# usamireko/WFL-ASR

Hardware: AMD Instinct MI355X
Metric: audio_seconds_labeled_per_sec_per_node (higher is better)
Workload: dtype bf16; 1 GPU; BASELINE configs[1]: openai/whisper-base + 2 Conformer blocks, 16 x 30 s clips per GPU; clips_per_gpu=16, frames_per_clip=1500, tags=141, parallelism=clip-sharded dp1, launch=eager, batches_in_flight=2

## Files before the change

wfl-asr_amd/csrc/gemm_stream.hip:

```cpp
#include "common.h"
#include <cstdlib>
#include <cstring>
#include <type_traits>

#define SBK 32
#ifndef SNST
#define SNST 4
#endif

#ifndef SNCU
#define SNCU 256
#endif

typedef __attribute__((address_space(1))) const void* sgptr_t;
typedef __attribute__((address_space(3))) void* slptr_t;
typedef __attribute__((ext_vector_type(2))) __bf16 bf16x2;

static __device__ __forceinline__ void sglds(const bf16_t* g, char* l) {
  __builtin_amdgcn_global_load_lds((sgptr_t)g, (slptr_t)l, 16, 0, 0);
}
static __device__ __forceinline__ int sswz(int row) { return (-(row >> 2)) & 3; }
static __device__ __forceinline__ int xswz(int row) { return ((row >> 2) & 1) << 1; }
template <int N>
static __device__ __forceinline__ void wait_vm() { asm volatile("s_waitcnt vmcnt(%0)" ::"n"(N) : "memory"); }

#ifdef WFL_GEMM_STAMPS
#define SSTAMP(k) do { if (tid == 0 && p.stamps) { p.stamps[(long)blockIdx.x * 8 + (k)] = __builtin_amdgcn_s_memrealtime(); \
    if ((k) == 1) p.stamps[(long)blockIdx.x * 8 + 5] = __builtin_amdgcn_s_memtime(); \
    if ((k) == 2) p.stamps[(long)blockIdx.x * 8 + 6] = __builtin_amdgcn_s_memtime(); } } while (0)
#else
#define SSTAMP(k) do { } while (0)
#endif

template <int ACT, int MT, bool RES, int LNF, bool STATS, bool CONV, bool W8 = false, bool A8 = false, bool OUT8 = false, bool NOLO = false>
__global__ __launch_bounds__(512) void gemm_stream_kernel(GemmArgs p) {
  static_assert(!NOLO || CONV, "only the conv mode has an optional low half");
  static_assert(!CONV || (MT == 6 && !RES && LNF == 0 && !STATS), "conv mode: 192-row tiles, plain epilogue");
  static_assert(!W8 || (!CONV && MT == 6), "fp8 weights: plain 192-row mode");
  static_assert(!A8 || (!W8 && !CONV && MT == 6 && LNF == 0 && !STATS), "fp8 x fp8: the plain 192-row mode, no LayerNorm folding");
  static_assert(!OUT8 || (A8 && !RES), "fp8 output: the fp8 x fp8 kernel, no residual");
  constexpr int BMV = MT * 32;
#ifdef WFL_LAB_STB32
  constexpr int STB = 512 * SBK * 2;
  constexpr int WOFF = 256 * SBK * 2;
#else
  constexpr int STB = CONV ? 256 * SBK * 2 : BMV * SBK * 2 + 256 * SBK * (W8 ? 1 : 2);
  constexpr int WOFF = CONV ? 0 : BMV * SBK * 2;
#endif
  constexpr int AEXT = 224 * SBK * 2;
  constexpr int AOFF = SNST * STB;
  constexpr bool LOUT = RES || (CONV && !NOLO);
  constexpr int NSTORE = (LOUT ? 4 : 2) * MT + (STATS ? MT : 0);
  constexpr int SROW = 4;
  extern __shared__ __attribute__((aligned(16))) char smem[];
  float* stat_lds = (float*)(smem + SNST * STB + (CONV ? 2 * AEXT : 0));
  const int tid = threadIdx.x;
  const int lane = tid & 63;
  const int wid = __builtin_amdgcn_readfirstlane(tid >> 6);
  const int grp = wid >> 2, wq = wid & 3;
  const int g = lane >> 4, c = lane & 15;
  const int G = gridDim.x;

  SSTAMP(0);
  const int tiles_n = p.N / 256;
  const int tiles_m = (p.M + BMV - 1) / BMV;
  const int ntiles = tiles_m * tiles_n;
  const int nk = p.K / SBK;
  auto tile_of = [&](int v, int& m0, int& n0) __attribute__((always_inline)) {
    const int q = ntiles >> 3, r = ntiles & 7, x = v & 7, i = v >> 3;
    const int bid = (x < r ? x * (q + 1) : r * (q + 1) + (x - r) * q) + i;
    const int tm = bid / tiles_n;
    m0 = tm * BMV;
    n0 = (bid - tm * tiles_n) * 256;
  };
  const int wm = grp * (MT * 16), wn = wq * 64;

  const bool two_x = CONV ? wid < 6 : (MT == 8 || wid < 4);
  const int xg0 = CONV ? (wid < 6 ? wid * 2 : 12 + (wid - 6)) : ((MT == 8 || wid < 4) ? wid * 2 : 8 + (wid - 4));
  const int ntaps = CONV ? (p.tap_wrap > 0 ? p.tap_wrap : p.K / p.cin) : 1;
  const int nchunk = CONV ? p.cin / SBK : 1;
  const bf16_t* a_src[2];
  const bf16_t* w_src[2];
  const char* w8_src = nullptr;
  int pv = blockIdx.x, pkt = 0, issued = 0;
  int islot = 0;
  int ptap_k = 0;
  long pbase = 0;
  int ptap_i = 0, pseg = 0;
  auto next_tap = [&]() __attribute__((always_inline)) {
    ptap_k = 0;
    if (p.tap_wrap > 0 && ++ptap_i == p.tap_wrap) { ptap_i = 0; ++pseg; pbase = pseg == 1 ? p.seg_off : 0; }
    else pbase += p.tap_stride;
  };
  int pcc = 0, ptap = 0, pccg = 0;
  long pa_off = 0, pw_off = 0;
  auto set_src = [&](int v) __attribute__((always_inline)) {
    int m0, n0;
    tile_of(v, m0, n0);
    int lane = tid & 63;
    asm volatile("" : "+v"(lane));
#pragma unroll
    for (int i = 0; i < 2; ++i) {
      const int wrow = (wid * 2 + i) * 16 + (lane >> 2);
      const int xrow = (xg0 + i) * 16 + (lane >> 2);
      int am = m0 + xrow;
      const int am_max = CONV ? p.M - 1 + ntaps - 1 : p.M - 1;
      am = am < am_max ? am : am_max;
      a_src[i] = p.A + (long)am * p.lda + ((lane & 3) ^ (CONV ? xswz(xrow) : sswz(xrow))) * 8;
      w_src[i] = p.W + (long)(n0 + wrow) * p.K + ((lane & 3) ^ sswz(wrow)) * 8;
    }
    if (W8) {
      const int Gr = wid * 4 + (lane >> 4);
      const int ul = (lane & 15) ^ ((Gr & 1) | (((Gr >> 1) & 1) << 3));
      w8_src = (const char*)p.W + (long)(n0 + 8 * Gr + (ul >> 1)) * p.K + (ul & 1) * 16;
    }
  };
  set_src(pv);
  auto issue_stage = [&]() __attribute__((always_inline)) {
    if (CONV) {
      char* base = smem + islot * STB;
      islot = islot + 1 == SNST ? 0 : islot + 1;
      if (ptap == 0) {
        char* ab = smem + AOFF + (pccg & 1) * AEXT;
        sglds(a_src[0] + pa_off, ab + xg0 * 1024);
        if (two_x) sglds(a_src[1] + pa_off, ab + xg0 * 1024 + 1024);
      }
#pragma unroll
      for (int i = 0; i < 2; ++i) sglds(w_src[i] + ptap * p.cin + pw_off, base + wid * 2048 + i * 1024);
      ++issued;
      ++pkt;
      if (++ptap == ntaps) {
        ptap = 0; ++pcc; ++pccg;
        if (pcc == nchunk) { pcc = 0; ++pseg; }
        pa_off = (pseg == 1 ? p.seg_off : 0) + (long)pcc * SBK;
        pw_off = (long)pseg * ntaps * p.cin + (long)pcc * SBK;
      }
      return;
    }
    const long koff = pbase + ptap_k;
    char* base = smem + islot * STB;
    islot = islot + 1 == SNST ? 0 : islot + 1;
    sglds(a_src[0] + koff, base + xg0 * 1024);
    if (two_x) sglds(a_src[1] + koff, base + xg0 * 1024 + 1024);
    if (W8) {
      sglds((const bf16_t*)(w8_src + pkt * SBK), base + WOFF + wid * 1024);
    } else {
#pragma unroll
      for (int i = 0; i < 2; ++i) sglds(w_src[i] + pkt * SBK, base + WOFF + wid * 2048 + i * 1024);
    }
    ++issued;
    ++pkt;
    ptap_k += SBK;
    if (ptap_k == p.cin) next_tap();
  };
  int d_pkt = 0;
  char* d_base = nullptr;
  auto issue_stage_split = [&](auto ndc_c) __attribute__((always_inline)) {
    constexpr int NDC = decltype(ndc_c)::value;
    const long koff = pbase + ptap_k;
    char* base = smem + islot * STB;
    islot = islot + 1 == SNST ? 0 : islot + 1;
    sglds(a_src[0] + koff, base + xg0 * 1024);
    if (two_x) sglds(a_src[1] + koff, base + xg0 * 1024 + 1024);
    if (W8) {
      if (NDC == 0) sglds((const bf16_t*)(w8_src + pkt * SBK), base + WOFF + wid * 1024);
    } else {
#pragma unroll
      for (int i = 0; i < 2 - NDC; ++i) sglds(w_src[i] + pkt * SBK, base + WOFF + wid * 2048 + i * 1024);
    }
    d_pkt = pkt; d_base = base;
    ++issued;
    ++pkt;
    ptap_k += SBK;
    if (ptap_k == p.cin) next_tap();
  };
  auto issue_deferred = [&](int j, auto ndc_c) __attribute__((always_inline)) {
    constexpr int NDC = decltype(ndc_c)::value;
    if (W8) sglds((const bf16_t*)(w8_src + d_pkt * SBK), d_base + WOFF + wid * 1024);
    else sglds(w_src[2 - NDC + j] + d_pkt * SBK, d_base + WOFF + wid * 2048 + (2 - NDC + j) * 1024);
  };
  auto prefetch_one = [&]() __attribute__((always_inline)) {
    if (pv >= ntiles) return;
    issue_stage();
    if (pkt == nk) {
      pkt = 0; ptap_k = 0; pbase = 0; pcc = 0; ptap = 0; ptap_i = 0; pseg = 0; pa_off = 0; pw_off = 0;
      pv += G;
      if (pv < ntiles) set_src(pv);
    }
  };
  auto wait_stage = [&](int need, bool with_stores) __attribute__((always_inline)) {
    const int younger = issued - need - 1;
    if (younger < 0) return;
    constexpr int L2X = CONV ? 2 : (W8 ? 3 : 4), L1X = CONV ? 2 : (W8 ? 2 : 3);
    static_assert(SNST >= 3 && SNST <= 6, "ring depth");
#define WFL_WAITY(L)                                                                              \
    do {                                                                                          \
      if (SNST >= 6 && younger >= 4) { if (with_stores) wait_vm<4 * (L) + NSTORE>(); else wait_vm<4 * (L)>(); }       \
      else if (SNST >= 5 && younger >= 3) { if (with_stores) wait_vm<3 * (L) + NSTORE>(); else wait_vm<3 * (L)>(); }  \
      else if (younger >= 2) { if (with_stores) wait_vm<2 * (L) + NSTORE>(); else wait_vm<2 * (L)>(); }              \
      else if (younger == 1) { if (with_stores) wait_vm<(L) + NSTORE>(); else wait_vm<(L)>(); }                      \
      else { if (with_stores) wait_vm<NSTORE>(); else wait_vm<0>(); }                                                \
    } while (0)
    if (CONV || two_x) WFL_WAITY(L2X); else WFL_WAITY(L1X);
#undef WFL_WAITY
  };

  int w_off[4];
#pragma unroll
  for (int v = 0; v < 4; ++v) {
#ifdef WFL_LAB_NOPERM
    const int r = wn + 16 * v + c;
#else
    const int r = wn + 32 * (v >> 1) + 8 * (c >> 2) + 4 * (v & 1) + (c & 3);
#endif
    w_off[v] = W8 ? WOFF + (r >> 3) * 256 + ((((r & 7) * 4 + g) ^ (((r >> 3) & 1) << 1) ^ (((r >> 4) & 1) << 4)) << 3)
                  : WOFF + r * 64 + ((g ^ sswz(r)) << 4);
  }
  const int x_off = wm * 64 + c * 64 + ((g ^ sswz(c)) << 4);

  f32x4 acc[MT][4];
#pragma unroll
  for (int u = 0; u < MT; ++u)
#pragma unroll
    for (int v = 0; v < 4; ++v) acc[u][v] = (f32x4){0.f, 0.f, 0.f, 0.f};
  float sa1 = 0.f, sa2 = 0.f, sb1 = 0.f, sb2 = 0.f;

  auto epilogue = [&](int m0, int n0) __attribute__((always_inline)) {
    const int nb = n0 + wn + 8 * g;
    int mrow0 = m0 + wm + c;
    int sidx_w = (((grp * 4 + wq) * (MT * 16)) + c) * 2, sidx_g = ((grp * 4 * (MT * 16)) + c) * 2, sidx_l = (grp * (MT * 16) + c) * 2;
    asm volatile("" : "+v"(mrow0), "+v"(sidx_w), "+v"(sidx_g), "+v"(sidx_l));
    f32x4 bj[4], sj[4], cj[(W8 || A8) ? 4 : 1];
#pragma unroll
    for (int h = 0; h < 2; ++h)
#pragma unroll
      for (int q = 0; q < 2; ++q) {
#ifdef WFL_ABL_EPI_NOLOAD
        bj[2 * h + q] = (f32x4){0.f, 0.f, 0.f, 0.f};
        if (LNF) sj[2 * h + q] = (f32x4){1.f, 1.f, 1.f, 1.f};
        if (W8 || A8) cj[2 * h + q] = (f32x4){1.f, 1.f, 1.f, 1.f};
#else
        bj[2 * h + q] = p.bias ? *(const f32x4*)(p.bias + nb + 32 * h + 4 * q) : (f32x4){0.f, 0.f, 0.f, 0.f};
        if (LNF) sj[2 * h + q] = *(const f32x4*)(p.ln_s + nb + 32 * h + 4 * q);
        if (W8 || A8) cj[2 * h + q] = *(const f32x4*)(p.w8_scale + nb + 32 * h + 4 * q);
#endif
      }
    float sa[A8 ? MT : 1];
    if (A8) {
#pragma unroll
      for (int u = 0; u < MT; ++u) {
        int m = mrow0 + 16 * u;
        m = m < p.M ? m : p.M - 1;
        sa[u] = p.a8_scale ? p.a8_scale[p.a8_lead + m] : p.a8_static;
      }
    }
    int P_ = p.P, cpitch = p.c_pitch;
    asm volatile("" : "+s"(P_), "+s"(cpitch));
    const float invP = __builtin_amdgcn_rcpf((float)P_);
    int orow[MT];
#pragma unroll
    for (int u = 0; u < MT; ++u) {
      const int m = mrow0 + 16 * u;
      int b = (int)((float)m * invP);
      int t = m - b * P_;
      if (t < 0) { t += P_; --b; }
      if (t >= P_) { t -= P_; ++b; }
      orow[u] = (m < p.M && t < p.T) ? (int)p.c_lead + b * cpitch + t : -1;
    }
    if (p.clip_T) {
#pragma unroll
      for (int u = 0; u < MT; ++u)
        if (orow[u] >= 0) {
          const int m = mrow0 + 16 * u;
          int b = (int)((float)m * invP);
          int t = m - b * P_;
          if (t < 0) { t += P_; --b; }
          if (t >= P_) { t -= P_; ++b; }
          if (t >= p.clip_T[b]) orow[u] = -1;
        }
    }
    constexpr int RING = 3;
    bf16x8 rr[RES ? RING : 1][2], rl[RES ? RING : 1][2];
    const bf16_t* res_lo = p.res_lo ? p.res_lo : p.res;
    const float lo_scale = p.res_lo ? 1.f : 0.f;
    auto load_res = [&](int u, int slot) __attribute__((always_inline)) {
      const long r = orow[u] >= 0 ? orow[u] : p.c_lead;
#pragma unroll
      for (int h = 0; h < 2; ++h) {
#ifdef WFL_ABL_EPI_NOLOAD
        rr[slot][h] = (bf16x8){0, 0, 0, 0, 0, 0, 0, 0}; rl[slot][h] = rr[slot][h]; (void)r;
#else
        rr[slot][h] = *(const bf16x8*)(p.res + r * p.ldres + nb + 32 * h);
        rl[slot][h] = *(const bf16x8*)(res_lo + r * p.ldres + nb + 32 * h);
#endif
      }
    };
    if (RES) {
#pragma unroll
      for (int u = 0; u < RING && u < MT; ++u) load_res(u, u);
    }
    float mu[LNF ? MT : 1], rs[LNF ? MT : 1];
    if (LNF == 1) {
#pragma unroll
      for (int u = 0; u < MT; ++u) {
        const float2 s = *(const float2*)(stat_lds + sidx_l + u * 32);
        mu[u] = s.x;
        rs[u] = s.y;
      }
    }
    if (LNF == 2) {
      f32x4 sp[MT][2];
#pragma unroll
      for (int u = 0; u < MT; ++u) {
        int m = mrow0 + 16 * u;
        m = m < p.M ? m : p.M - 1;
        const f32x4* q = (const f32x4*)(p.stats_in + (p.stats_lead + m) * (2 * SROW));
        sp[u][0] = q[0];
        sp[u][1] = q[1];
      }
#pragma unroll
      for (int u = 0; u < MT; ++u) {
        float a1 = sp[u][0][0], a2 = sp[u][0][1];
        if (p.stats_nsl > 1) { a1 += sp[u][0][2]; a2 += sp[u][0][3]; }
        if (p.stats_nsl > 2) { a1 += sp[u][1][0]; a2 += sp[u][1][1]; }
        if (p.stats_nsl > 3) { a1 += sp[u][1][2]; a2 += sp[u][1][3]; }
        float mean, ex2;
        if (p.ln_k_pow2) { mean = a1 * p.ln_inv_k; ex2 = a2 * p.ln_inv_k; }
        else { mean = a1 / (float)p.K; ex2 = a2 / (float)p.K; }
        mu[u] = mean;
        rs[u] = rsqrtf(fmaxf(__builtin_fmaf(-mean, mean, ex2), 0.f) + p.ln_eps);
      }
    }
    char* trash = (char*)p.trash + lane * 16;
#ifdef WFL_ABL_EPI_NOSTORE
#define WFL_KEEP(k) false
#else
#define WFL_KEEP(k) (k)
#endif
    float t1 = 0.f, t2 = 0.f;
    float amax8 = 0.f;
#pragma unroll
    for (int u = 0; u < MT; ++u) {
      __builtin_amdgcn_sched_barrier(0);
#pragma unroll
      for (int h = 0; h < 2; ++h) {
        float x[8];
#pragma unroll
        for (int q = 0; q < 2; ++q)
#pragma unroll
          for (int e = 0; e < 4; ++e) {
            float v = acc[u][2 * h + q][e];
            if (W8 || A8) v *= cj[2 * h + q][e];
            if (A8) v *= sa[u];
            if (LNF) v = (v - mu[u] * sj[2 * h + q][e]) * rs[u];
            if (ACT == WFL_ACT_GELU) {
              x[4 * q + e] = v + bj[2 * h + q][e];
              if (e & 1) {
                const f32x2 y = gelu_erf2((f32x2){x[4 * q + e - 1], x[4 * q + e]});
                x[4 * q + e - 1] = y[0]; x[4 * q + e] = y[1];
              }
              continue;
            }
            v = apply_act<ACT>(v + bj[2 * h + q][e]);
            if (RES) v = (bf2f(rr[u % RING][h][4 * q + e]) + lo_scale * bf2f(rl[u % RING][h][4 * q + e])) + p.alpha * v;
            x[4 * q + e] = v;
          }
        bf16x8 o;
#pragma unroll
        for (int e = 0; e < 8; ++e) o[e] = f2bf(x[e]);
        const bool keep = orow[u] >= 0 && nb + 32 * h < p.n_valid;
        if (OUT8) {
          int w0 = 0, w1 = 0;
          const float keepf = keep ? 1.f : 0.f;
#pragma unroll
          for (int e = 0; e < 8; ++e) {
            const float y = x[e] * p.c8_inv_scale;
            amax8 = fmaxf(amax8, fabsf(y) * keepf);
            x[e] = fminf(fmaxf(y, -448.f), 448.f);
          }
          w0 = __builtin_amdgcn_cvt_pk_fp8_f32(x[0], x[1], w0, false); w0 = __builtin_amdgcn_cvt_pk_fp8_f32(x[2], x[3], w0, true);
          w1 = __builtin_amdgcn_cvt_pk_fp8_f32(x[4], x[5], w1, false); w1 = __builtin_amdgcn_cvt_pk_fp8_f32(x[6], x[7], w1, true);
          char* d8 = (char*)(p.c8 + (long)orow[u] * p.ldc8 + nb + 32 * h);
          d8 = WFL_KEEP(keep) ? d8 : trash;
          *(uint2*)d8 = make_uint2((unsigned)w0, (unsigned)w1);
          continue;
        }
        char* dst = (char*)((bf16_t*)p.C + (long)orow[u] * p.ldc + nb + 32 * h);
        dst = WFL_KEEP(keep) ? dst : trash;
        *(bf16x8*)dst = o;
        if (LOUT) {
          bf16x8 ol;
#pragma unroll
          for (int e = 0; e < 8; ++e) ol[e] = f2bf(x[e] - bf2f(o[e]));
          char* dl = (char*)(p.c_lo + (long)orow[u] * p.ldc + nb + 32 * h);
          dl = WFL_KEEP(keep && p.c_lo) ? dl : trash;
          *(bf16x8*)dl = ol;
        }
        if (STATS) {
#pragma unroll
          for (int e = 0; e < 8; ++e) { const float r = bf2f(o[e]); t1 += r; t2 = fmaf(r, r, t2); }
        }
      }
      if (STATS) {
        t1 += __shfl_xor(t1, 16); t2 += __shfl_xor(t2, 16);
        t1 += __shfl_xor(t1, 32); t2 += __shfl_xor(t2, 32);
        if (g == 0) *(float2*)(stat_lds + sidx_w + u * 32) = float2{t1, t2};
        t1 = t2 = 0.f;
      }
#pragma unroll
      for (int v = 0; v < 4; ++v) acc[u][v] = (f32x4){0.f, 0.f, 0.f, 0.f};
      if (RES && u + RING < MT) load_res(u + RING, u % RING);
    }
    if (OUT8 && p.err) {
      if (__builtin_amdgcn_ballot_w64(amax8 > 448.f) && lane == 0) atomicOr(p.err, 2u);
    }
    if (STATS) {
      unsigned* cnt = (unsigned*)(stat_lds + 8 * (MT * 16) * 2) + grp;
      __builtin_amdgcn_s_waitcnt(0xC07F);
      unsigned ticket = 0;
      if (lane == 0) ticket = atomicAdd(cnt, 1u);
      ticket = __builtin_amdgcn_readfirstlane(ticket);
      const bool last = ticket == 3;
      if (last && lane == 0) *cnt = 0;
#pragma unroll
      for (int u = 0; u < MT; ++u) {
        float a1 = 0.f, a2 = 0.f;
#pragma unroll
        for (int w4 = 0; w4 < 4; ++w4) {
          const float2 v = *(const float2*)(stat_lds + sidx_g + w4 * (MT * 32) + u * 32);
          a1 += v.x; a2 += v.y;
        }
        float* sd = p.stats_out + ((long)orow[u] * SROW + (n0 >> 8)) * 2;
        sd = (last && orow[u] >= 0 && g == 0) ? sd : (float*)trash;
        *(float2*)sd = float2{a1, a2};
      }
    }
  };

  if (STATS && tid < 2) ((unsigned*)(stat_lds + 8 * (MT * 16) * 2))[tid] = 0;
#pragma unroll
  for (int t = 0; t < SNST - 1; ++t) prefetch_one();
  wait_stage(0, false);
  __builtin_amdgcn_s_barrier();
  SSTAMP(1);
  if (grp) __builtin_amdgcn_s_barrier();

#define SSB() __builtin_amdgcn_sched_barrier(0)
  bf16x8 fw[4], fx[MT];
#ifndef WFL_W8_CVT_IN_C
#define WFL_W8_CVT_IN_C 1
#endif
  uint2 fraw[W8 ? 4 : 1];
  int s = 0;
  int rslot = 0;
  int ctap = 0, ccg = 0;
  auto read_frags = [&]() __attribute__((always_inline)) {
    const char* sb = smem + rslot * STB;
    if (W8 && WFL_W8_CVT_IN_C) {
#pragma unroll
      for (int v = 0; v < 4; ++v) fraw[v] = *(const uint2*)(sb + w_off[v]);
    } else if (W8) {
#pragma unroll
      for (int v = 0; v < 4; ++v) {
        const uint2 raw = *(const uint2*)(sb + w_off[v]);
        const bf16x2 a = __builtin_amdgcn_cvt_scalef32_pk_bf16_fp8(raw.x, 1.0f, false), b = __builtin_amdgcn_cvt_scalef32_pk_bf16_fp8(raw.x, 1.0f, true);
        const bf16x2 c2 = __builtin_amdgcn_cvt_scalef32_pk_bf16_fp8(raw.y, 1.0f, false), d2 = __builtin_amdgcn_cvt_scalef32_pk_bf16_fp8(raw.y, 1.0f, true);
        fw[v] = (bf16x8){a[0], a[1], b[0], b[1], c2[0], c2[1], d2[0], d2[1]};
      }
    } else {
#pragma unroll
      for (int v = 0; v < 4; ++v) fw[v] = *(const bf16x8*)(sb + w_off[v]);
    }
    if (CONV) {
      const char* ab = smem + AOFF + (ccg & 1) * AEXT;
      const int r0 = wm + c + ctap;
      const int xb = r0 * 64 + ((g ^ xswz(r0)) << 4);
#pragma unroll
      for (int u = 0; u < MT; ++u) fx[u] = *(const bf16x8*)(ab + xb + u * 1024);
      if (++ctap == ntaps) { ctap = 0; ++ccg; }
      return;
    }
#pragma unroll
    for (int u = 0; u < MT; ++u) fx[u] = *(const bf16x8*)(sb + x_off + u * 1024);
  };
  auto mma_all = [&](auto ndc_c) __attribute__((always_inline)) {
    constexpr int NDC = decltype(ndc_c)::value;
    const bf16x2 one2 = {(bf16_t)1.0f, (bf16_t)1.0f};
#pragma unroll
    for (int u = 0; u < MT; ++u) {
#pragma unroll
      for (int v = 0; v < 4; ++v) {
        if (W8 && WFL_W8_CVT_IN_C && u == 0) {
          const uint2 raw = fraw[v];
          const bf16x2 a = __builtin_amdgcn_cvt_scalef32_pk_bf16_fp8(raw.x, 1.0f, false), b = __builtin_amdgcn_cvt_scalef32_pk_bf16_fp8(raw.x, 1.0f, true);
          const bf16x2 c2 = __builtin_amdgcn_cvt_scalef32_pk_bf16_fp8(raw.y, 1.0f, false), d2 = __builtin_amdgcn_cvt_scalef32_pk_bf16_fp8(raw.y, 1.0f, true);
          fw[v] = (bf16x8){a[0], a[1], b[0], b[1], c2[0], c2[1], d2[0], d2[1]};
        }
        if (A8) {
          typedef __attribute__((ext_vector_type(2))) long i64x2;
          const i64x2 a = __builtin_bit_cast(i64x2, fw[v]), b = __builtin_bit_cast(i64x2, fx[u]);
          acc[u][v] = __builtin_amdgcn_mfma_f32_16x16x32_fp8_fp8(a[0], b[0], acc[u][v], 0, 0, 0);
          acc[u][v] = __builtin_amdgcn_mfma_f32_16x16x32_fp8_fp8(a[1], b[1], acc[u][v], 0, 0, 0);
        } else acc[u][v] = __builtin_amdgcn_mfma_f32_16x16x32_bf16(fw[v], fx[u], acc[u][v], 0, 0, 0);
      }
      if (NDC >= 1 && u == 1) { __builtin_amdgcn_sched_barrier(0); issue_deferred(0, ndc_c); __builtin_amdgcn_sched_barrier(0); }
      if (NDC >= 2 && u == 3) { __builtin_amdgcn_sched_barrier(0); issue_deferred(1, ndc_c); __builtin_amdgcn_sched_barrier(0); }
      if (LNF == 1) {
        if ((u & 3) == wq) {
#pragma unroll
          for (int j = 0; j < 4; ++j) {
            const bf16x2 xv = {fx[u][2 * j], fx[u][2 * j + 1]};
            if (u < 4) {
              sa1 = __builtin_amdgcn_fdot2_f32_bf16(xv, one2, sa1, false);
              sa2 = __builtin_amdgcn_fdot2_f32_bf16(xv, xv, sa2, false);
            } else {
              sb1 = __builtin_amdgcn_fdot2_f32_bf16(xv, one2, sb1, false);
              sb2 = __builtin_amdgcn_fdot2_f32_bf16(xv, xv, sb2, false);
            }
          }
        }
      }
    }
  };
  auto ln_publish = [&]() __attribute__((always_inline)) {
#pragma unroll
    for (int i = 0; i < 2; ++i) {
      float a1 = i ? sb1 : sa1, a2 = i ? sb2 : sa2;
      a1 += __shfl_xor(a1, 16); a2 += __shfl_xor(a2, 16);
      a1 += __shfl_xor(a1, 32); a2 += __shfl_xor(a2, 32);
      const float mean = a1 / (float)p.K;
      const float var = fmaxf(a2 / (float)p.K - mean * mean, 0.f);
      const int u = wq + 4 * i;
      if (u < MT && g == 0) {
        float2 o = {mean, rsqrtf(var + p.ln_eps)};
        *(float2*)(stat_lds + (grp * (MT * 16) + u * 16 + c) * 2) = o;
      }
    }
    sa1 = sa2 = sb1 = sb2 = 0.f;
  };
  int pm0 = 0, pn0 = 0;
  bool have_prev = false;
  for (int tv = blockIdx.x; tv < ntiles; tv += G) {
    int m0, n0;
    tile_of(tv, m0, n0);
    const bool last_tile = tv + G >= ntiles;
    auto step_general = [&](int kt, auto first_c) __attribute__((always_inline)) {
      if (decltype(first_c)::value && have_prev) epilogue(pm0, pn0);
      read_frags();
      prefetch_one();
      if (grp) wait_stage(s + 1, have_prev && kt < SNST - 2);
      __builtin_amdgcn_s_waitcnt(0xC07F);
      __builtin_amdgcn_s_barrier();
      SSB();
      mma_all(std::integral_constant<int, 0>{});
      if (LNF == 1 && kt == nk - 1) ln_publish();
      SSB();
      if (!grp) wait_stage(s + 1, have_prev && kt < SNST - 2);
      if (LNF == 1) __builtin_amdgcn_s_waitcnt(0xC07F);
      if (LNF == 1 || !(grp && last_tile && kt == nk - 1)) __builtin_amdgcn_s_barrier();
      SSB();
      ++s;
      rslot = rslot + 1 == SNST ? 0 : rslot + 1;
    };
    auto steps_steady = [&](auto grp_c) __attribute__((always_inline)) {
      constexpr bool GRP1 = decltype(grp_c)::value;
      constexpr int NL = CONV ? 2 : ((MT == 8 || !GRP1) ? (W8 ? 3 : 4) : (W8 ? 2 : 3));
#ifndef WFL_DMA_IN_C
#define WFL_DMA_IN_C 0
#endif
      constexpr int NDC = CONV ? 0 : (W8 ? (WFL_DMA_IN_C > 1 ? 1 : WFL_DMA_IN_C) : WFL_DMA_IN_C);
      const std::integral_constant<int, NDC> ndc_c{};
      for (int kt = SNST - 2; kt <= nk - SNST - 1; ++kt) {
#ifndef WFL_ABL_NOLDS
        read_frags();
#endif
#ifndef WFL_ABL_NOSTAGE
        if (CONV) issue_stage(); else issue_stage_split(ndc_c);
#else
        ++issued; ++pkt; if (CONV) { if (++ptap == ntaps) { ptap = 0; ++pcc; ++pccg; } }
#endif
        if (GRP1) wait_vm<(SNST - 2) * NL - NDC>();
        __builtin_amdgcn_s_waitcnt(0xC07F);
        __builtin_amdgcn_s_barrier();
        SSB();
        mma_all(ndc_c);
        SSB();
        if (!GRP1) wait_vm<(SNST - 2) * NL>();
        __builtin_amdgcn_s_barrier();
        SSB();
        ++s;
        rslot = rslot + 1 == SNST ? 0 : rslot + 1;
      }
    };
    step_general(0, std::true_type{});
#pragma unroll
    for (int kt = 1; kt < SNST - 2; ++kt) step_general(kt, std::false_type{});
    if (grp) steps_steady(std::true_type{}); else steps_steady(std::false_type{});
    for (int kt = nk - SNST > SNST - 2 ? nk - SNST : SNST - 2; kt < nk; ++kt) step_general(kt, std::false_type{});
    pm0 = m0; pn0 = n0;
    have_prev = true;
  }
  SSTAMP(2);
  SSTAMP(3);
  if (have_prev) epilogue(pm0, pn0);
  if (LNF == 1 && !grp) __builtin_amdgcn_s_barrier();
  SSTAMP(4);
#undef SSB
}

template <int ACT, int MT, bool RES, int LNF, bool STATS, bool CONV = false, bool W8 = false, bool A8 = false, bool OUT8 = false, bool NOLO = false>
static int launch_stream(const GemmArgs& a, hipStream_t s) {
  constexpr int BMV = MT * 32;
#ifdef WFL_LAB_STB32
  constexpr int lds = SNST * 512 * SBK * 2 + 8 * (MT * 16) * 2 * 4 + 64;
#else
  constexpr int lds = (CONV ? SNST * 256 * SBK * 2 + 2 * 224 * SBK * 2 : SNST * (BMV * SBK * 2 + 256 * SBK * (W8 ? 1 : 2))) + 8 * (MT * 16) * 2 * 4 + 64;
#endif
  const int tiles = ((a.M + BMV - 1) / BMV) * (a.N / 256);
  auto k = gemm_stream_kernel<ACT, MT, RES, LNF, STATS, CONV, W8, A8, OUT8, NOLO>;
  static WflOncePerDevice attr_once;
  if (attr_once.need()) {
    if (hipFuncSetAttribute((const void*)k, hipFuncAttributeMaxDynamicSharedMemorySize, lds) != hipSuccess) return -2;
  }
  g_wfl_gemm_kernel_id = CONV ? 6 : ((W8 || A8) ? 7 : (MT == 6 ? 1 : 5));
  hipLaunchKernelGGL(k, dim3(tiles < SNCU ? tiles : SNCU), dim3(512), lds, s, a);
  return hipGetLastError() == hipSuccess ? 0 : -3;
}

template <int ACT, bool RES, int LNF, bool STATS = false>
static int launch_stream_mt(const GemmArgs& a, hipStream_t s) {
  static int forced = -1;
  if (forced < 0) { const char* e = getenv("WFL_GEMM_BM"); forced = e ? atoi(e) : 0; }
#ifdef WFL_STREAM_MT8
  if (forced == 256) return launch_stream<ACT, 8, RES, LNF, STATS>(a, s);
#endif
  return launch_stream<ACT, 6, RES, LNF, STATS>(a, s);
}

static bool wfl_gemm_stream_conv(const GemmArgs& a) {
  static int off = -1;
  if (off < 0) { const char* e = getenv("WFL_GEMM_NO_CONV"); off = e && atoi(e) ? 1 : 0; }
  if (off) return false;
  const int taps = a.tap_wrap > 0 ? a.tap_wrap : a.K / a.cin;
  if (a.tap_wrap > 0 && a.K != 3 * a.tap_wrap * a.cin) return false;
  return a.cin < a.K && a.K % a.cin == 0 && taps <= 32 && taps >= SNST - 1 && a.tap_stride == a.lda && a.cin % SBK == 0 &&
         !a.res && !a.ln_s && !a.stats_out;
}

bool wfl_gemm_stream_conv_takes(const GemmArgs& a);
bool wfl_gemm_stream_takes(const GemmArgs& a) {
  static int off = -1;
  if (off < 0) { const char* e = getenv("WFL_GEMM_NO_STREAM"); off = e && atoi(e) ? 1 : 0; }
  if (off) return false;
#ifdef WFL_LAB_NOSTREAM
  return false;
#endif
  if (a.glu || a.out_f32 || a.pos || a.clip_bias) return false;
  if (a.a8 >= 2) return false;
  if (a.tap_wrap > 0 && (a.ln_s || a.w8_scale || a.a8)) return false;
  if (a.c_lo && !a.res && !wfl_gemm_stream_conv(a)) return false;
  if (a.w8_scale && (a.cin < a.K || a.K % 64)) return false;
  if (a.a8 && (!a.w8_scale || a.ln_s || a.stats_out || a.stats_in || a.K % 128 || a.lda % 16 || a.K / 64 < 8 || (a.c8 && (a.res || a.ldc8 % 8))))
    return false;
  if (a.c8 && !a.a8) return false;
  if (a.N % 256 || a.K % SBK || a.cin % SBK || a.K / SBK < 8 || a.n_valid % 8) return false;
  if (a.stats_out && (!a.res || a.N / 256 > 4)) return false;
  if (a.stats_in && (!a.ln_s || a.stats_nsl <= 0 || a.stats_nsl > 4)) return false;
  if (a.res && a.act != WFL_ACT_NONE) return false;
  if (a.ln_s && (a.res || a.cin < a.K || (a.act != WFL_ACT_NONE && a.act != WFL_ACT_GELU))) return false;
  if (a.act == WFL_ACT_SIGMOID) return false;
  return true;
}


bool wfl_gemm_stream_conv_takes(const GemmArgs& a) { return wfl_gemm_stream_takes(a) && wfl_gemm_stream_conv(a); }

int wfl_launch_gemm_stream(const GemmArgs& a, hipStream_t s) {
  if (!wfl_gemm_stream_takes(a)) return 1;
  static void* trash[32] = {nullptr};
  int dev = 0;
  (void)hipGetDevice(&dev);
  dev &= 31;
  if (!trash[dev]) {
    if (hipMalloc(&trash[dev], 4096) != hipSuccess) return -2;
  }
  GemmArgs g = a;
  g.trash = trash[dev];
  g.ln_k_pow2 = (g.K & (g.K - 1)) == 0;
  g.ln_inv_k = g.ln_k_pow2 ? 1.0f / (float)g.K : 0.f;
  if (g.a8) {
    g.K /= 2; g.cin = g.K; g.lda /= 2;
    if (g.c8) return g.act == WFL_ACT_GELU ? launch_stream<WFL_ACT_GELU, 6, false, 0, false, false, false, true, true>(g, s) : -1;
    if (g.res) return g.act == WFL_ACT_NONE ? launch_stream<WFL_ACT_NONE, 6, true, 0, false, false, false, true>(g, s) : -1;
    if (g.act == WFL_ACT_NONE) return launch_stream<WFL_ACT_NONE, 6, false, 0, false, false, false, true>(g, s);
    return -1;
  }
  if (g.w8_scale) {
    if (g.ln_s && g.stats_in) {
      if (g.act == WFL_ACT_NONE) return launch_stream<WFL_ACT_NONE, 6, false, 2, false, false, true>(g, s);
      if (g.act == WFL_ACT_GELU) return launch_stream<WFL_ACT_GELU, 6, false, 2, false, false, true>(g, s);
      return -1;
    }
    if (g.res && !g.ln_s && g.act == WFL_ACT_NONE)
      return g.stats_out ? launch_stream<WFL_ACT_NONE, 6, true, 0, true, false, true>(g, s)
                         : launch_stream<WFL_ACT_NONE, 6, true, 0, false, false, true>(g, s);
    if (!g.res && !g.ln_s) {
      if (g.act == WFL_ACT_NONE) return launch_stream<WFL_ACT_NONE, 6, false, 0, false, false, true>(g, s);
      if (g.act == WFL_ACT_GELU) return launch_stream<WFL_ACT_GELU, 6, false, 0, false, false, true>(g, s);
    }
    return -1;
  }
  if (g.ln_s) {
    if (g.stats_in) {
      switch (g.act) {
        case WFL_ACT_NONE: return launch_stream_mt<WFL_ACT_NONE, false, 2>(g, s);
        case WFL_ACT_GELU: return launch_stream_mt<WFL_ACT_GELU, false, 2>(g, s);
      }
      return 1;
    }
    switch (g.act) {
      case WFL_ACT_NONE: return launch_stream_mt<WFL_ACT_NONE, false, 1>(g, s);
      case WFL_ACT_GELU: return launch_stream_mt<WFL_ACT_GELU, false, 1>(g, s);
    }
    return 1;
  }
  if (wfl_gemm_stream_conv(g)) {
    if (!g.c_lo) {
      switch (g.act) {
        case WFL_ACT_NONE: return launch_stream<WFL_ACT_NONE, 6, false, 0, false, true, false, false, false, true>(g, s);
        case WFL_ACT_GELU: return launch_stream<WFL_ACT_GELU, 6, false, 0, false, true, false, false, false, true>(g, s);
        case WFL_ACT_RELU: return launch_stream<WFL_ACT_RELU, 6, false, 0, false, true, false, false, false, true>(g, s);
      }
      return 1;
    }
    switch (g.act) {
      case WFL_ACT_NONE: return launch_stream<WFL_ACT_NONE, 6, false, 0, false, true>(g, s);
      case WFL_ACT_GELU: return launch_stream<WFL_ACT_GELU, 6, false, 0, false, true>(g, s);
      case WFL_ACT_RELU: return launch_stream<WFL_ACT_RELU, 6, false, 0, false, true>(g, s);
    }
    return 1;
  }
  if (g.res) return g.stats_out ? launch_stream_mt<WFL_ACT_NONE, true, 0, true>(g, s) : launch_stream_mt<WFL_ACT_NONE, true, 0>(g, s);
  switch (g.act) {
    case WFL_ACT_NONE: return launch_stream_mt<WFL_ACT_NONE, false, 0>(g, s);
    case WFL_ACT_GELU: return launch_stream_mt<WFL_ACT_GELU, false, 0>(g, s);
    case WFL_ACT_RELU: return launch_stream_mt<WFL_ACT_RELU, false, 0>(g, s);
  }
  return 1;
}
```

Measured before the change: 134,500 audio-s/s.

## Rotate frame fragments across conv taps to reuse LDS reads in conv GEMM

Adds a ROT mode to the conv-streaming GEMM that lays frame rows out contiguously in LDS (223-row chunks) and assigns each lane MT consecutive frames. Across taps the already-loaded fragments shift by one register, so only the newest fragment is read from LDS per tap. The epilogue row mapping and weight fragment offsets change to match. It is on by default through the WFL_CONV_ROTATE env var, and it risks extra register moves, LDS bank conflicts from the new layout, and correctness issues in the index remapping.

Result: faster. 136,000 audio-s/s (median of 6 runs) (+1.1%).

```diff
diff --git a/wfl-asr_amd/csrc/gemm_stream.hip b/wfl-asr_amd/csrc/gemm_stream.hip
--- a/wfl-asr_amd/csrc/gemm_stream.hip
+++ b/wfl-asr_amd/csrc/gemm_stream.hip
@@ -21,6 +21,7 @@
 }
 static __device__ __forceinline__ int sswz(int row) { return (-(row >> 2)) & 3; }
 static __device__ __forceinline__ int xswz(int row) { return ((row >> 2) & 1) << 1; }
+#define XROT_ROWS 223
 template <int N>
 static __device__ __forceinline__ void wait_vm() { asm volatile("s_waitcnt vmcnt(%0)" ::"n"(N) : "memory"); }
 
@@ -32,9 +33,10 @@
 #define SSTAMP(k) do { } while (0)
 #endif
 
-template <int ACT, int MT, bool RES, int LNF, bool STATS, bool CONV, bool W8 = false, bool A8 = false, bool OUT8 = false, bool NOLO = false>
+template <int ACT, int MT, bool RES, int LNF, bool STATS, bool CONV, bool W8 = false, bool A8 = false, bool OUT8 = false, bool NOLO = false, bool ROT = false>
 __global__ __launch_bounds__(512) void gemm_stream_kernel(GemmArgs p) {
   static_assert(!NOLO || CONV, "only the conv mode has an optional low half");
+  static_assert(!ROT || CONV, "only the conv mode rotates frame fragments");
   static_assert(!CONV || (MT == 6 && !RES && LNF == 0 && !STATS), "conv mode: 192-row tiles, plain epilogue");
   static_assert(!W8 || (!CONV && MT == 6), "fp8 weights: plain 192-row mode");
   static_assert(!A8 || (!W8 && !CONV && MT == 6 && LNF == 0 && !STATS), "fp8 x fp8: the plain 192-row mode, no LayerNorm folding");
@@ -102,11 +104,13 @@
 #pragma unroll
     for (int i = 0; i < 2; ++i) {
       const int wrow = (wid * 2 + i) * 16 + (lane >> 2);
-      const int xrow = (xg0 + i) * 16 + (lane >> 2);
+      const int xslot = (xg0 + i) * 64 + lane;
+      const int xch = (xslot >= XROT_ROWS) + (xslot >= 2 * XROT_ROWS) + (xslot >= 3 * XROT_ROWS);
+      const int xrow = ROT ? xslot - XROT_ROWS * xch : (xg0 + i) * 16 + (lane >> 2);
       int am = m0 + xrow;
       const int am_max = CONV ? p.M - 1 + ntaps - 1 : p.M - 1;
       am = am < am_max ? am : am_max;
-      a_src[i] = p.A + (long)am * p.lda + ((lane & 3) ^ (CONV ? xswz(xrow) : sswz(xrow))) * 8;
+      a_src[i] = p.A + (long)am * p.lda + (ROT ? xch : (lane & 3) ^ (CONV ? xswz(xrow) : sswz(xrow))) * 8;
       w_src[i] = p.W + (long)(n0 + wrow) * p.K + ((lane & 3) ^ sswz(wrow)) * 8;
     }
     if (W8) {
@@ -227,7 +231,8 @@
 
   auto epilogue = [&](int m0, int n0) __attribute__((always_inline)) {
     const int nb = n0 + wn + 8 * g;
-    int mrow0 = m0 + wm + c;
+    constexpr int FCOL = ROT ? MT : 1, FROW = ROT ? 1 : 16;
+    int mrow0 = m0 + wm + FCOL * c;
     int sidx_w = (((grp * 4 + wq) * (MT * 16)) + c) * 2, sidx_g = ((grp * 4 * (MT * 16)) + c) * 2, sidx_l = (grp * (MT * 16) + c) * 2;
     asm volatile("" : "+v"(mrow0), "+v"(sidx_w), "+v"(sidx_g), "+v"(sidx_l));
     f32x4 bj[4], sj[4], cj[(W8 || A8) ? 4 : 1];
@@ -249,7 +254,7 @@
     if (A8) {
 #pragma unroll
       for (int u = 0; u < MT; ++u) {
-        int m = mrow0 + 16 * u;
+        int m = mrow0 + FROW * u;
         m = m < p.M ? m : p.M - 1;
         sa[u] = p.a8_scale ? p.a8_scale[p.a8_lead + m] : p.a8_static;
       }
@@ -260,7 +265,7 @@
     int orow[MT];
 #pragma unroll
     for (int u = 0; u < MT; ++u) {
-      const int m = mrow0 + 16 * u;
+      const int m = mrow0 + FROW * u;
       int b = (int)((float)m * invP);
       int t = m - b * P_;
       if (t < 0) { t += P_; --b; }
@@ -271,7 +276,7 @@
 #pragma unroll
       for (int u = 0; u < MT; ++u)
         if (orow[u] >= 0) {
-          const int m = mrow0 + 16 * u;
+          const int m = mrow0 + FROW * u;
           int b = (int)((float)m * invP);
           int t = m - b * P_;
           if (t < 0) { t += P_; --b; }
@@ -312,7 +317,7 @@
       f32x4 sp[MT][2];
 #pragma unroll
       for (int u = 0; u < MT; ++u) {
-        int m = mrow0 + 16 * u;
+        int m = mrow0 + FROW * u;
         m = m < p.M ? m : p.M - 1;
         const f32x4* q = (const f32x4*)(p.stats_in + (p.stats_lead + m) * (2 * SROW));
         sp[u][0] = q[0];
@@ -454,7 +459,7 @@
   int s = 0;
   int rslot = 0;
   int ctap = 0, ccg = 0;
-  auto read_frags = [&]() __attribute__((always_inline)) {
+  auto read_frags = [&](bool carry) __attribute__((always_inline)) {
     const char* sb = smem + rslot * STB;
     if (W8 && WFL_W8_CVT_IN_C) {
 #pragma unroll
@@ -469,7 +474,18 @@
       }
     } else {
 #pragma unroll
-      for (int v = 0; v < 4; ++v) fw[v] = *(const bf16x8*)(sb + w_off[v]);
+      for (int v = 0; v < 4; ++v) fw[v] = ROT ? *(const bf16x8*)(sb + w_off[v & 1] + (v >> 1) * 2048) : *(const bf16x8*)(sb + w_off[v]);
+    }
+    if (ROT) {
+      const char* ab = smem + AOFF + (ccg & 1) * AEXT;
+      const int xb = (XROT_ROWS * g + wm + MT * c + ctap) * 16;
+      if (!carry || ctap == 0) {
+#pragma unroll
+        for (int u = 0; u < MT - 1; ++u) fx[u] = *(const bf16x8*)(ab + xb + u * 16);
+      }
+      fx[MT - 1] = *(const bf16x8*)(ab + xb + (MT - 1) * 16);
+      if (++ctap == ntaps) { ctap = 0; ++ccg; }
+      return;
     }
     if (CONV) {
       const char* ab = smem + AOFF + (ccg & 1) * AEXT;
@@ -503,6 +519,12 @@
           acc[u][v] = __builtin_amdgcn_mfma_f32_16x16x32_fp8_fp8(a[1], b[1], acc[u][v], 0, 0, 0);
         } else acc[u][v] = __builtin_amdgcn_mfma_f32_16x16x32_bf16(fw[v], fx[u], acc[u][v], 0, 0, 0);
       }
+      if (ROT && u + 1 < MT) {
+        typedef __attribute__((ext_vector_type(4))) int i32x4;
+        i32x4 t = __builtin_bit_cast(i32x4, fx[u + 1]);
+        asm volatile("" : "+v"(t));
+        fx[u] = __builtin_bit_cast(bf16x8, t);
+      }
       if (NDC >= 1 && u == 1) { __builtin_amdgcn_sched_barrier(0); issue_deferred(0, ndc_c); __builtin_amdgcn_sched_barrier(0); }
       if (NDC >= 2 && u == 3) { __builtin_amdgcn_sched_barrier(0); issue_deferred(1, ndc_c); __builtin_amdgcn_sched_barrier(0); }
       if (LNF == 1) {
@@ -546,7 +568,7 @@
     const bool last_tile = tv + G >= ntiles;
     auto step_general = [&](int kt, auto first_c) __attribute__((always_inline)) {
       if (decltype(first_c)::value && have_prev) epilogue(pm0, pn0);
-      read_frags();
+      read_frags(false);
       prefetch_one();
       if (grp) wait_stage(s + 1, have_prev && kt < SNST - 2);
       __builtin_amdgcn_s_waitcnt(0xC07F);
@@ -572,7 +594,7 @@
       const std::integral_constant<int, NDC> ndc_c{};
       for (int kt = SNST - 2; kt <= nk - SNST - 1; ++kt) {
 #ifndef WFL_ABL_NOLDS
-        read_frags();
+        read_frags(ROT && kt > SNST - 2);
 #endif
 #ifndef WFL_ABL_NOSTAGE
         if (CONV) issue_stage(); else issue_stage_split(ndc_c);
@@ -608,7 +630,7 @@
 #undef SSB
 }
 
-template <int ACT, int MT, bool RES, int LNF, bool STATS, bool CONV = false, bool W8 = false, bool A8 = false, bool OUT8 = false, bool NOLO = false>
+template <int ACT, int MT, bool RES, int LNF, bool STATS, bool CONV = false, bool W8 = false, bool A8 = false, bool OUT8 = false, bool NOLO = false, bool ROT = false>
 static int launch_stream(const GemmArgs& a, hipStream_t s) {
   constexpr int BMV = MT * 32;
 #ifdef WFL_LAB_STB32
@@ -617,7 +639,7 @@
   constexpr int lds = (CONV ? SNST * 256 * SBK * 2 + 2 * 224 * SBK * 2 : SNST * (BMV * SBK * 2 + 256 * SBK * (W8 ? 1 : 2))) + 8 * (MT * 16) * 2 * 4 + 64;
 #endif
   const int tiles = ((a.M + BMV - 1) / BMV) * (a.N / 256);
-  auto k = gemm_stream_kernel<ACT, MT, RES, LNF, STATS, CONV, W8, A8, OUT8, NOLO>;
+  auto k = gemm_stream_kernel<ACT, MT, RES, LNF, STATS, CONV, W8, A8, OUT8, NOLO, ROT>;
   static WflOncePerDevice attr_once;
   if (attr_once.need()) {
     if (hipFuncSetAttribute((const void*)k, hipFuncAttributeMaxDynamicSharedMemorySize, lds) != hipSuccess) return -2;
@@ -648,6 +670,24 @@
 }
 
 bool wfl_gemm_stream_conv_takes(const GemmArgs& a);
+
+template <bool ROT>
+static int launch_conv(const GemmArgs& g, hipStream_t s) {
+  if (!g.c_lo) {
+    switch (g.act) {
+      case WFL_ACT_NONE: return launch_stream<WFL_ACT_NONE, 6, false, 0, false, true, false, false, false, true, ROT>(g, s);
+      case WFL_ACT_GELU: return launch_stream<WFL_ACT_GELU, 6, false, 0, false, true, false, false, false, true, ROT>(g, s);
+      case WFL_ACT_RELU: return launch_stream<WFL_ACT_RELU, 6, false, 0, false, true, false, false, false, true, ROT>(g, s);
+    }
+    return 1;
+  }
+  switch (g.act) {
+    case WFL_ACT_NONE: return launch_stream<WFL_ACT_NONE, 6, false, 0, false, true, false, false, false, false, ROT>(g, s);
+    case WFL_ACT_GELU: return launch_stream<WFL_ACT_GELU, 6, false, 0, false, true, false, false, false, false, ROT>(g, s);
+    case WFL_ACT_RELU: return launch_stream<WFL_ACT_RELU, 6, false, 0, false, true, false, false, false, false, ROT>(g, s);
+  }
+  return 1;
+}
 bool wfl_gemm_stream_takes(const GemmArgs& a) {
   static int off = -1;
   if (off < 0) { const char* e = getenv("WFL_GEMM_NO_STREAM"); off = e && atoi(e) ? 1 : 0; }
@@ -725,20 +765,9 @@
     return 1;
   }
   if (wfl_gemm_stream_conv(g)) {
-    if (!g.c_lo) {
-      switch (g.act) {
-        case WFL_ACT_NONE: return launch_stream<WFL_ACT_NONE, 6, false, 0, false, true, false, false, false, true>(g, s);
-        case WFL_ACT_GELU: return launch_stream<WFL_ACT_GELU, 6, false, 0, false, true, false, false, false, true>(g, s);
-        case WFL_ACT_RELU: return launch_stream<WFL_ACT_RELU, 6, false, 0, false, true, false, false, false, true>(g, s);
-      }
-      return 1;
-    }
-    switch (g.act) {
-      case WFL_ACT_NONE: return launch_stream<WFL_ACT_NONE, 6, false, 0, false, true>(g, s);
-      case WFL_ACT_GELU: return launch_stream<WFL_ACT_GELU, 6, false, 0, false, true>(g, s);
-      case WFL_ACT_RELU: return launch_stream<WFL_ACT_RELU, 6, false, 0, false, true>(g, s);
-    }
-    return 1;
+    const char* e = getenv("WFL_CONV_ROTATE");
+    const bool rot = !(e && e[0] == '0' && !e[1]);
+    return rot ? launch_conv<true>(g, s) : launch_conv<false>(g, s);
   }
   if (g.res) return g.stats_out ? launch_stream_mt<WFL_ACT_NONE, true, 0, true>(g, s) : launch_stream_mt<WFL_ACT_NONE, true, 0>(g, s);
   switch (g.act) {
```
